# kishwarshafin/pepper

Measured on AMD Instinct MI355X. Metric: inference windows/sec (whole node), higher is better.
Workload: dtype f32 via f16 hi/lo split operands (3 MFMAs per product), f32 accumulate

## Files before the change

### include/pepper_amd_debug.h

```cpp
#ifndef PEPPER_AMD_DEBUG_H
#define PEPPER_AMD_DEBUG_H

#ifdef __cplusplus
extern "C" {
#endif

int pa_debug_dump_timing(unsigned long long* host_out);
int pa_debug_dump_gru_timing(unsigned long long* host_out);
void pa_debug_gemm_h2_experiment(int e);
int pa_debug_gemm_h2(const float* A, const float* W, const float* bias, float* C, int a_rows, int M, int N, int K, int act,
                     int frag_T, int frag_nb, int iters, float* ms_out);
int pa_debug_gemm_h2_split(const float* A, const float* W, const float* bias, float* C_new, float* C_parent, int a_rows, int M,
                           int N, int K, int act, int splits, int iters, float* ms_new, float* ms_parent);

#ifdef __cplusplus
}
#endif
#endif
```

### pepper_amd/csrc/api.hip

```cpp
#include "../../include/pepper_amd.h"

#include <hip/hip_runtime.h>

#include <algorithm>
#include <cmath>
#include <cstdio>
#include <cstdlib>
#include <cstring>
#include <map>
#include <string>
#include <vector>

#include "dec_frag16.h"
#include "kernels.h"

namespace {
thread_local std::string g_err;
}

namespace pa {
int set_error(int code, const std::string& msg) {
    g_err = msg;
    return code;
}
// ... 680 lines not shown
        HIP_TRY(hipMemsetAsync(m->us_failed->p, 0, sizeof(int), m->stream));
        HIP_TRY(hipMemcpyAsync(&m->us_host[1], ovf_counter, sizeof(int), hipMemcpyDeviceToHost, m->stream));
    }
    const size_t xp_bytes = std::max(s.need_xp ? (size_t)np * T * NX * sizeof(float) : (size_t)0,
                                     (size_t)8 * n * m->L1 * sizeof(float));
    if (int rc = m->xp->ensure(xp_bytes)) return rc;
    if (int rc = m->ya->ensure((size_t)np * T * 2 * H * sizeof(float))) return rc;
    if (m->rec.size() > 1)
        if (int rc = m->yb->ensure((size_t)np * T * 2 * H * sizeof(float))) return rc;
    if (int rc = m->l1->ensure((size_t)n * m->L1 * sizeof(float))) return rc;
    if (int rc = m->l2->ensure((size_t)n * m->L1 * sizeof(float))) return rc;
    const int tiles1 = (int)((n + 255) / 256) * ((m->L1 + 255) / 256);
    while (!bi && s.l1_splits < 32 && tiles1 * s.l1_splits * 2 <= 256 &&
           (size_t)(s.l1_splits * 2) * n * m->L1 * sizeof(float) <= m->xp->bytes)
        s.l1_splits *= 2;
    if (bi) s.l1_splits = kCanonicalL1Splits;

    const void* cur = images;
    int cur_kind = a_kind, cur_ld = F;
    bool cur_h2 = false;
    float* ybuf[2] = {m->ya->f(), m->yb->f()};
    int which = 0;
    const int M = (int)(n * T);
    for (size_t li = 0; li < m->rec.size(); ++li) {
        const RecLayer& r = m->rec[li];
        const LayerForm<Rec>& f = forms[li];
        float* y = ybuf[which];
        const float* bias_l = (f.y_h2 && r.prescaled) ? r.b_in_s->f() : r.b_in->f();
        const float* wih_l = (f.y_h2 && r.prescaled) ? r.w_ih_s->f() : r.w_ih->f();
        if (f.proj == XP_GEMM_H2) {
            const size_t a_bytes = (size_t)M * cur_ld * sizeof(float);
            if (!cur_h2)
                LAUNCH_TRY(m, "cvt_h2", 0.0,
                           pa::launch_f32_to_h2(static_cast<const float*>(cur), const_cast<void*>(cur), M, r.K,
                                                cur_ld, m->stream));
            LAUNCH_TRY(m, "gemm_h2_inproj", 2.0 * M * NX * r.K,
                       pa::launch_gemm_h2(cur, cur_ld, a_bytes, r.w_ih_h2->p, r.K, (size_t)NX * r.K * 4, bias_l,
                                          m->xp->f(), NX, (int)(np * T), NX, r.K, 0, 0, 0, T, (int)n, m->stream));
        } else if (f.proj == XP_GEMM_F32) {
            LAUNCH_TRY(m, li == 0 ? "gemm_inproj_in" : "gemm_inproj", 2.0 * M * NX * r.K,
                       pa::launch_gemm_nt(cur_kind, cur, cur_ld, wih_l, r.Kp, bias_l, m->xp->f(),
                                          NX, (int)(np * T), NX, r.K, 0, 0, 0, T, (int)n, m->stream));
        }
        switch (f.rec) {
        case FUSED_IN_H2:
            LAUNCH_TRY(m, "lstm_rec_h2_fused_in", 2.0 * n * T * (4.0 * H) * (H + r.K) * 2,
                       pa::launch_lstm_enc_h2(H, static_cast<const int8_t*>(cur), r.K, bias_l, r.w_cat_h2->p, y, 2 * H, (int)n, T,
                                              m->stream, s.small_rows));
            break;
        case FUSED_IN_F32:
            LAUNCH_TRY(m, "lstm_rec_fused_in", 2.0 * n * T * (4.0 * H) * (H + r.K) * 2,
                       pa::launch_lstm_rec_fused(H, static_cast<const int8_t*>(cur), r.K, r.b_in->f(),
                                                 r.w_cat->f(), y, 2 * H, (int)n, T, m->stream));
            break;
        case FUSED_DEC_H2:
            LAUNCH_TRY(m, "lstm_dec_h2_fused", 2.0 * n * T * (4.0 * H) * (H + r.K) * 2,
                       pa::launch_lstm_dec_h2(H, cur, cur_ld, bias_l, r.w_cat_dec_h2->p, y, 2 * H, (int)n, T, m->stream,
                                              bi && s.small_rows));
            break;
        case SPLIT_H2: {
            const int sabotage = m->split_sabotage > 0 ? 1 : 0;
            m->split_sabotage -= sabotage;
            LAUNCH_TRY(m, "lstm_rec_h2_split", 2.0 * n * T * (4.0 * H) * H * 2,
                       pa::launch_lstm_rec_h2_split(H, m->xp->f(), NX, r.w_hh_h2->p, y, 2 * H, (int)n, T, m->us_exch->p,
                                                    m->us_cnt->p, static_cast<int*>(m->us_failed->p), m->stream, sabotage));
            break;
        }
        case PLAIN_H2:
            LAUNCH_TRY(m, "lstm_rec_h2", 2.0 * n * T * (4.0 * H) * H * 2,
                       pa::launch_lstm_seed_h2(H, m->xp->f(), NX, r.w_hh_h2->p, y, 2 * H, (int)n, T, m->stream, s.small_rows));
            break;
        case PLAIN_F32:
            LAUNCH_TRY(m, "lstm_rec", 2.0 * n * T * (4.0 * H) * H * 2,
                       pa::launch_lstm_rec(H, m->xp->f(), NX, r.w_hh->f(), y, 2 * H, (int)n, T, m->stream));
            break;
        }
        cur = y;
        cur_kind = pa::A_F32;
        cur_ld = 2 * H;
        cur_h2 = f.y_h2;
        which ^= 1;
    }
    const int K1 = T * 2 * H;
    if (m->split_gemm && m->lin[0].w_h2 != nullptr && cur_kind == pa::A_F32) {
        if (!cur_h2)
            LAUNCH_TRY(m, "cvt_h2", 0.0,
                       pa::launch_f32_to_h2(static_cast<const float*>(cur), const_cast<void*>(cur), n, K1, K1, m->stream));
        LAUNCH_TRY(m, "gemm_h2_linear_1", 2.0 * n * m->L1 * K1,
                   pa::launch_gemm_h2(cur, K1, (size_t)n * K1 * 4, m->lin[0].w_h2->p, K1, (size_t)m->L1 * K1 * 4,
                                      m->lin[0].b->f(), m->l1->f(), m->L1, (int)n, m->L1, K1, 1, 0, 0, 0, 0, m->stream,
                                      s.l1_splits > 1 ? m->xp->f() : nullptr, s.l1_splits));
    } else {
        LAUNCH_TRY(m, "gemm_linear_1", 2.0 * n * m->L1 * K1,
                   pa::launch_gemm_nt(pa::A_F32, cur, K1, m->lin[0].w->f(), K1, m->lin[0].b->f(), m->l1->f(),
                                      m->L1, (int)n, m->L1, K1, 1, 0, 0, 0, 0, m->stream));
    }
    if (m->mlp_w != nullptr && C <= 8) {
        LAUNCH_TRY(m, "mlp_tail_h2", 2.0 * n * m->L1 * (4.0 * m->L1 + C),
                   pa::launch_mlp_tail_h2(m->l1->f(), m->L1, m->mlp_w->p, m->mlp_b->f(), 4, m->out.w->f(), m->out.b->f(), C,
                                          probs, logits, (int)n, m->stream, static_cast<const float* const*>(m->mlp_w32->p),
                                          ovf_counter, bi));
        if (s.unit_split) {
            HIP_TRY(hipMemcpyAsync(&m->us_host[0], m->us_failed->p, sizeof(int), hipMemcpyDeviceToHost, m->stream));
            HIP_TRY(hipStreamSynchronize(m->stream));
            if (m->us_host[0] != 0) {
                ++m->split_fallbacks;
                m->split_holdoff = US_HOLDOFF;
                HIP_TRY(hipMemcpyAsync(ovf_counter, &m->us_host[1], sizeof(int), hipMemcpyHostToDevice, m->stream));
                return variant_forward_chunk(m, a_kind, images, n, probs, logits, false);
            }
        }
        return PA_OK;
    }
    float* a = m->l1->f();
    float* b = m->l2->f();
    for (int i = 1; i < 5; ++i) {
        LAUNCH_TRY(m, "gemm_linear_2to5", 2.0 * n * m->L1 * m->L1,
                   pa::launch_gemm_nt(pa::A_F32, a, m->L1, m->lin[i].w->f(), m->L1, m->lin[i].b->f(), b,
                                      m->L1, (int)n, m->L1, m->L1, 1, 0, 0, 0, 0, m->stream));
        std::swap(a, b);
    }
    LAUNCH_TRY(m, "head_softmax", 2.0 * n * m->L1 * C,
               pa::launch_dense_small(0, a, m->L1, m->out.w->f(), m->out.b->f(), probs, logits, (int)n,
                                      m->L1, C, 1, 1, 0, m->stream));
    return PA_OK;
}

static int variant_forward(pa_variant_model* m, int a_kind, const void* images, size_t elem, int64_t n,
                           float* probs, float* logits) {
    if (!as_base(m)) return fail(PA_ERR_INVALID, "bad model handle");
    if (n < 0 || (n > 0 && (!images || !probs))) return fail(PA_ERR_INVALID, "null buffer");
    HIP_TRY(hipSetDevice(m->device));
    const int64_t per = (int64_t)m->cfg.window * m->cfg.image_features;
    const int C = m->cfg.num_classes_type;
    for (int64_t off = 0; off < n; off += m->cfg.max_chunk) {
        const int64_t c = std::min<int64_t>(m->cfg.max_chunk, n - off);
        const char* img = static_cast<const char*>(images) + (size_t)off * per * elem;
        if (int rc = variant_forward_chunk(m, a_kind, img, c, probs + off * C,
                                           logits ? logits + off * C : nullptr))
            return rc;
    }
    return PA_OK;
}

int pa_variant_split_fallbacks(pa_variant_model* m, int64_t* calls) {
    if (!as_base(m) || !calls) return fail(PA_ERR_INVALID, "bad argument");
    *calls = m->split_fallbacks;
    return PA_OK;
}

int pa_variant_set_batch_invariant(pa_variant_model* m, int32_t on) {
    return set_batch_invariant(m, on, "pa_variant_set_batch_invariant");
}

int pa_variant_get_batch_invariant(pa_variant_model* m, int32_t* on) { return get_batch_invariant(m, on); }

int pa_variant_overflow_rows(pa_variant_model* m, int64_t* rows) {
    if (!as_base(m) || !rows) return fail(PA_ERR_INVALID, "bad model handle");
    HIP_TRY(hipSetDevice(m->device));
    int v = 0;
    if (m->mlp_w32 != nullptr) {
        HIP_TRY(hipStreamSynchronize(m->stream));
        HIP_TRY(hipMemcpy(&v, m->ovf_counter(), sizeof(int), hipMemcpyDeviceToHost));
    }
    *rows = v;
    return PA_OK;
}

int pa_variant_forward_device(pa_variant_model* m, const int8_t* images, int64_t n, float* probs,
                              float* logits) {
    return variant_forward(m, pa::A_I8, images, 1, n, probs, logits);
}

int pa_variant_forward_device_f32(pa_variant_model* m, const float* images, int64_t n, float* probs,
                                  float* logits) {
    return variant_forward(m, pa::A_F32_SCALAR, images, 4, n, probs, logits);
}

int pa_variant_forward_host(pa_variant_model* m, const int8_t* images, int64_t n, float* probs,
                            float* logits) {
    if (!as_base(m)) return fail(PA_ERR_INVALID, "bad model handle");
    if (n < 0 || (n > 0 && (!images || !probs))) return fail(PA_ERR_INVALID, "null buffer");
    if (n == 0) return PA_OK;
    const size_t per = (size_t)m->cfg.window * m->cfg.image_features;
// ... 428 lines not shown
```

### pepper_amd/csrc/gemm_h2.hip

```cpp
#include "common.h"
#include "kernels.h"

#include <cstdlib>
#include <vector>

namespace {

typedef _Float16 h8 __attribute__((ext_vector_type(8)));

constexpr int HM = 256, HN = 256, HK = 32;
constexpr int HROW = 36;
constexpr int HSTAGE = (HM + HN) * HROW;

PA_DEV f32x16 mfma_h(h8 a, h8 b, f32x16 c) { return __builtin_amdgcn_mfma_f32_32x32x16_f16(a, b, c, 0, 0, 0); }

template <int ACT, int EXP = 0>
__global__ __launch_bounds__(256) void gemm_h2_kernel(const uint32_t* __restrict__ A, int lda, uint32_t a_bytes,
                                                      const uint32_t* __restrict__ W, int ldw, uint32_t w_bytes,
                                                      const float* __restrict__ bias, float* __restrict__ C, int ldc,
                                                      int M, int N, int K, int tiles_n, int nwg, int a_rpb,
                                                      int64_t a_bstride, int frag_T, int frag_nb) {
    __shared__ __attribute__((aligned(16))) uint32_t lds[2 * HSTAGE];

    const int tile = xcd_swizzle(blockIdx.x, nwg);
// ... 298 lines not shown
    int lane_ep = lane;
    asm volatile("" : "+v"(lane_ep));
    const int row_ep = m0 + wm * 128 + (lane_ep & 15), col_ep = n0 + wn * 128 + 4 * (lane_ep >> 4);
#pragma unroll
    for (int m = 0; m < 8; ++m) {
        const int row = row_ep + m * 16;
#pragma unroll
        for (int n = 0; n < 8; ++n) {
            const int col = col_ep + n * 16;
            if (row < M && col < N) *reinterpret_cast<f32x4*>(C + (size_t)row * N + col) = acc[m][n];
        }
    }
}

template <int ACT>
__global__ __launch_bounds__(256) void splitk_finish_kernel(const float* __restrict__ part, int S, const float* __restrict__ bias,
                                                            float* __restrict__ C, int ldc, int M, int N) {
    const size_t idx = (size_t)blockIdx.x * 256 + threadIdx.x;
    const int n4 = N >> 2;
    if (idx >= (size_t)M * n4) return;
    const int row = (int)(idx / n4), c = (int)(idx % n4) * 4;
    f32x4 v = *reinterpret_cast<const f32x4*>(part + (size_t)row * N + c);
    for (int s = 1; s < S; ++s) {
        const f32x4 w = *reinterpret_cast<const f32x4*>(part + ((size_t)s * M + row) * N + c);
        v += w;
    }
    if (bias != nullptr) v += *reinterpret_cast<const f32x4*>(bias + c);
    if (ACT == 1) { v.x = selu_f(v.x); v.y = selu_f(v.y); v.z = selu_f(v.z); v.w = selu_f(v.w); }
    *reinterpret_cast<f32x4*>(C + (size_t)row * ldc + c) = v;
}

__global__ __launch_bounds__(256) void f32_to_h2_kernel(const float* __restrict__ src, uint32_t* __restrict__ dst,
                                                        int64_t rows, int K, int64_t ld) {
    const int64_t idx = (int64_t)blockIdx.x * 256 + threadIdx.x;
    const int gpr = K >> 3;
    if (idx >= rows * gpr) return;
    const int64_t r = idx / gpr;
    const int g = (int)(idx - r * gpr);
    const float* s = src + r * ld + g * 8;
    h8 hi, lo;
#pragma unroll
    for (int e = 0; e < 8; ++e) {
        hi[e] = (_Float16)s[e];
        lo[e] = (_Float16)(s[e] - (float)hi[e]);
    }
    h8* d = reinterpret_cast<h8*>(dst + r * ld + g * 8);
    d[0] = hi;
    d[1] = lo;
}

}

namespace pa {

static bool g_h2_split_parent = false;
int g_h2_exp = 0;

void split_h2_host(const float* src, uint32_t* dst, int64_t rows, int K, int64_t ld_src, int64_t ld_dst) {
    for (int64_t r = 0; r < rows; ++r) {
        const float* s = src + r * ld_src;
        _Float16* d = reinterpret_cast<_Float16*>(dst + r * ld_dst);
        for (int g = 0; g < K / 8; ++g)
            for (int e = 0; e < 8; ++e) {
                const float v = s[g * 8 + e];
                const _Float16 hi = (_Float16)v;
                d[g * 16 + e] = hi;
                d[g * 16 + 8 + e] = (_Float16)(v - (float)hi);
            }
    }
}

hipError_t launch_f32_to_h2(const float* src, void* dst, int64_t rows, int K, int64_t ld, hipStream_t stream) {
    if ((K & 7) || (ld & 7)) return hipErrorInvalidValue;
    const int64_t n = rows * (K >> 3);
    if (n == 0) return hipSuccess;
    hipLaunchKernelGGL(f32_to_h2_kernel, dim3((unsigned)((n + 255) / 256)), dim3(256), 0, stream, src,
                       reinterpret_cast<uint32_t*>(dst), rows, K, ld);
    return hipGetLastError();
}

hipError_t launch_gemm_h2(const void* A, int lda, size_t a_bytes, const void* W, int ldw, size_t w_bytes,
                          const float* bias, float* C, int ldc, int M, int N, int K, int act, int a_rpb,
                          int64_t a_bstride, int frag_T, int frag_nb, hipStream_t stream, float* splitk_ws,
                          int splits) {
    if (frag_T > 0 && ((M & 31) || (N & 31) || act != 0)) return hipErrorInvalidValue;
    if ((K % HK) || (lda & 7) || (ldw & 7) || (a_bstride & 7) || ((uintptr_t)A & 15) || ((uintptr_t)W & 15))
        return hipErrorInvalidValue;
    if (a_bytes >= (1ull << 32) || w_bytes >= (1ull << 32)) return hipErrorInvalidValue;
    const int tiles_m = (M + HM - 1) / HM, tiles_n = (N + HN - 1) / HN;
    const int nwg = tiles_m * tiles_n;
    if (nwg == 0) return hipSuccess;
    const uint32_t* Au = reinterpret_cast<const uint32_t*>(A);
    const uint32_t* Wu = reinterpret_cast<const uint32_t*>(W);
    if (splits > 1 && splitk_ws != nullptr && frag_T == 0 && !(N & 3) && K / HK >= splits) {
        if (g_h2_split_parent)
            hipLaunchKernelGGL((gemm_h2_kernel<0>), dim3(nwg, splits), dim3(256), 0, stream, Au, lda, (uint32_t)a_bytes, Wu,
                               ldw, (uint32_t)w_bytes, (const float*)nullptr, splitk_ws, N, M, N, K, tiles_n, nwg, a_rpb,
                               a_bstride, 0, 0);
        else
            hipLaunchKernelGGL(gemm_h2_k32_kernel, dim3(nwg, splits), dim3(256), 0, stream, Au, lda, (uint32_t)a_bytes, Wu,
                               ldw, (uint32_t)w_bytes, splitk_ws, M, N, K, tiles_n, nwg, a_rpb, a_bstride);
        const size_t n4 = (size_t)M * (N >> 2);
        if (act == 1)
            hipLaunchKernelGGL((splitk_finish_kernel<1>), dim3((unsigned)((n4 + 255) / 256)), dim3(256), 0, stream,
                               splitk_ws, splits, bias, C, ldc, M, N);
        else
            hipLaunchKernelGGL((splitk_finish_kernel<0>), dim3((unsigned)((n4 + 255) / 256)), dim3(256), 0, stream,
                               splitk_ws, splits, bias, C, ldc, M, N);
        return hipGetLastError();
    }
    if (g_h2_exp > 0 && g_h2_exp < 8) {
#define PA_EXP(E_) case E_: hipLaunchKernelGGL((gemm_h2_kernel<0, E_>), dim3(nwg), dim3(256), 0, stream, Au, lda, (uint32_t)a_bytes, Wu, ldw, (uint32_t)w_bytes, bias, C, ldc, M, N, K, tiles_n, nwg, a_rpb, a_bstride, frag_T, frag_nb); break;
        switch (g_h2_exp) { PA_EXP(1) PA_EXP(2) PA_EXP(3) PA_EXP(4) PA_EXP(5) PA_EXP(6) PA_EXP(7) }
#undef PA_EXP
        return hipGetLastError();
    }
    if (act == 1)
        hipLaunchKernelGGL((gemm_h2_kernel<1>), dim3(nwg), dim3(256), 0, stream, Au, lda, (uint32_t)a_bytes, Wu, ldw,
                           (uint32_t)w_bytes, bias, C, ldc, M, N, K, tiles_n, nwg, a_rpb, a_bstride, frag_T, frag_nb);
    else
        hipLaunchKernelGGL((gemm_h2_kernel<0>), dim3(nwg), dim3(256), 0, stream, Au, lda, (uint32_t)a_bytes, Wu, ldw,
                           (uint32_t)w_bytes, bias, C, ldc, M, N, K, tiles_n, nwg, a_rpb, a_bstride, frag_T, frag_nb);
    return hipGetLastError();
}

}

extern "C" void pa_debug_gemm_h2_experiment(int e) { pa::g_h2_exp = e; }

extern "C" int pa_debug_gemm_h2(const float* A, const float* W, const float* bias, float* C, int a_rows, int M, int N,
                                int K, int act, int frag_T, int frag_nb, int iters, float* ms_out) {
    void *dA = nullptr, *dA2 = nullptr, *dW = nullptr, *dB = nullptr, *dC = nullptr;
    const size_t a_bytes = (size_t)a_rows * K * 4, w_bytes = (size_t)N * K * 4;
    const size_t c_elems = frag_T > 0 ? (size_t)M * N : (size_t)M * N;
    std::vector<uint32_t> wh((size_t)N * K);
    pa::split_h2_host(W, wh.data(), N, K, K, K);
    hipError_t e = hipSuccess;
    auto ok = [&](hipError_t r) { if (e == hipSuccess) e = r; return r == hipSuccess; };
    ok(hipMalloc(&dA, a_bytes)); ok(hipMalloc(&dA2, a_bytes)); ok(hipMalloc(&dW, w_bytes));
    ok(hipMalloc(&dB, (size_t)N * 4)); ok(hipMalloc(&dC, c_elems * 4));
    if (e == hipSuccess) {
        ok(hipMemcpy(dA, A, a_bytes, hipMemcpyHostToDevice));
        ok(hipMemcpy(dW, wh.data(), w_bytes, hipMemcpyHostToDevice));
        if (bias) ok(hipMemcpy(dB, bias, (size_t)N * 4, hipMemcpyHostToDevice));
        ok(hipMemset(dC, 0, c_elems * 4));
        ok(pa::launch_f32_to_h2((const float*)dA, dA2, a_rows, K, K, nullptr));
        hipEvent_t e0, e1;
        ok(hipEventCreate(&e0)); ok(hipEventCreate(&e1));
        ok(pa::launch_gemm_h2(dA2, K, a_bytes, dW, K, w_bytes, bias ? (const float*)dB : nullptr, (float*)dC, N, M, N, K,
                              act, 0, 0, frag_T, frag_nb, nullptr));
        ok(hipDeviceSynchronize());
        ok(hipEventRecord(e0, nullptr));
        for (int i = 0; i < iters; ++i)
            ok(pa::launch_gemm_h2(dA2, K, a_bytes, dW, K, w_bytes, bias ? (const float*)dB : nullptr, (float*)dC, N, M, N,
                                  K, act, 0, 0, frag_T, frag_nb, nullptr));
        ok(hipEventRecord(e1, nullptr));
        ok(hipEventSynchronize(e1));
        float ms = 0.0f;
        ok(hipEventElapsedTime(&ms, e0, e1));
        if (ms_out) *ms_out = iters > 0 ? ms / iters : 0.0f;
        ok(hipMemcpy(C, dC, c_elems * 4, hipMemcpyDeviceToHost));
        (void)hipEventDestroy(e0);
        (void)hipEventDestroy(e1);
    }
    for (void* p : {(void*)dA, (void*)dA2, (void*)dW, (void*)dB, (void*)dC}) (void)hipFree(p);
    if (e != hipSuccess) return pa::set_error((int)e, std::string("pa_debug_gemm_h2: ") + hipGetErrorString(e));
    return 0;
}

extern "C" int pa_debug_gemm_h2_split(const float* A, const float* W, const float* bias, float* C_new, float* C_parent,
                                      int a_rows, int M, int N, int K, int act, int splits, int iters, float* ms_new,
                                      float* ms_parent) {
    if (splits < 2 || (N & 3) || K % HK || K / HK < splits || a_rows < 1 || M < 1)
        return pa::set_error((int)hipErrorInvalidValue, "pa_debug_gemm_h2_split: needs splits >= 2, N % 4 == 0, K / 32 >= splits");
    void *dA = nullptr, *dA2 = nullptr, *dW = nullptr, *dB = nullptr, *dC = nullptr, *dWs = nullptr;
    const size_t a_bytes = (size_t)a_rows * K * 4, w_bytes = (size_t)N * K * 4, c_elems = (size_t)M * N;
    std::vector<uint32_t> wh((size_t)N * K);
    pa::split_h2_host(W, wh.data(), N, K, K, K);
    hipError_t e = hipSuccess;
    auto ok = [&](hipError_t r) { if (e == hipSuccess) e = r; return r == hipSuccess; };
    ok(hipMalloc(&dA, a_bytes)); ok(hipMalloc(&dA2, a_bytes)); ok(hipMalloc(&dW, w_bytes));
    ok(hipMalloc(&dB, (size_t)N * 4)); ok(hipMalloc(&dC, c_elems * 4)); ok(hipMalloc(&dWs, c_elems * 4 * splits));
    if (e == hipSuccess) {
        ok(hipMemcpy(dA, A, a_bytes, hipMemcpyHostToDevice));
// ... 33 lines not shown
```

### pepper_amd/csrc/kernels.h

```cpp
#pragma once
#include <hip/hip_runtime.h>
#include <stdint.h>

#include <string>

namespace pa {

int set_error(int code, const std::string& msg);

enum AKind { A_F32 = 0, A_I8 = 1, A_U8 = 2, A_F32_SCALAR = 3 };

hipError_t launch_gemm_nt(int a_type, const void* A, int lda, const float* W, int ldw,
                          const float* bias, float* C, int ldc, int M, int N, int K, int act,
                          int a_rpb, int64_t a_bstride, int frag_T, int frag_nb, hipStream_t stream);

hipError_t launch_gemm_h2(const void* A, int lda, size_t a_bytes, const void* W, int ldw, size_t w_bytes,
                          const float* bias, float* C, int ldc, int M, int N, int K, int act, int a_rpb,
                          int64_t a_bstride, int frag_T, int frag_nb, hipStream_t stream,
                          float* splitk_ws = nullptr, int splits = 1);
hipError_t launch_f32_to_h2(const float* src, void* dst, int64_t rows, int K, int64_t ld, hipStream_t stream);
void split_h2_host(const float* src, uint32_t* dst, int64_t rows, int K, int64_t ld_src, int64_t ld_dst);

hipError_t launch_lstm_rec(int H, const float* Xp, int ldx, const float* Wp, float* Y, int ldy,
                           int B, int T, hipStream_t stream);
hipError_t launch_lstm_rec_fused(int H, const int8_t* X, int F, const float* bias, const float* Wcat,
                                 float* Y, int ldy, int B, int T, hipStream_t stream);
hipError_t launch_gru_rec(int H, const float* Xp, int ldx, const float* Wp, const float* bhn,
                          const float* h0, int ldh0, float* hn, int ldhn, float* Y, int ldy,
                          int B, int T, hipStream_t stream);

hipError_t launch_gru_rec_fused(int H, const uint8_t* X, int F, int64_t x_bstride, const float* bias,
                                const float* Wcat, const float* bhn, const float* h0, int ldh0, float* hn, int ldhn,
                                float* Y, int ldy, int B, int T, hipStream_t stream);

void pack_rec_weights_h2(const float* const whh[2], const float* const wih[2], int G, int H, int F, int KX,
                         uint32_t* out, const float* const* bias = nullptr);
size_t rec_weights_h2_words(int G, int H, int KX);
int gru_fused_input_kx(int H, int F);
hipError_t launch_lstm_seed_h2(int H, const float* Xp, int ldx, const void* Wp, void* Y, int ldy, int B, int T,
                               hipStream_t stream, bool small = false);
hipError_t launch_lstm_enc_h2(int H, const int8_t* X, int F, const float* bias, const void* Wp, void* Y, int ldy, int B, int T,
                              hipStream_t stream, bool small = false);

size_t lstm_split_exchange_bytes(int B);
size_t lstm_split_counter_bytes(int B);
int lstm_split_grid(int B);
int lstm_split_resident_workgroups(int ntw);
hipError_t launch_lstm_rec_h2_split(int H, const float* Xp, int ldx, const void* Wp, void* Y, int ldy, int B, int T, void* exch,
                                    void* counters, int* failed, hipStream_t stream, int sabotage = 0);

hipError_t launch_lstm_dec_h2(int H, const void* Xh, int ldxh, const float* bias, const void* Wp, void* Y, int ldy, int B,
                              int T, hipStream_t stream, bool small = false);
hipError_t launch_gru_rec_h2(int H, const float* Xp, int ldx, const uint8_t* X, int F, int64_t x_bstride,
                             const float* bias, const void* Wp, const float* bhn, const float* h0, int ldh0, float* hn,
                             int ldhn, void* Y, int ldy, int B, int T, hipStream_t stream);

void pack_gru_small_weights_h2(const float* const whh[2], int H, uint32_t* out);
size_t gru_small_weights_h2_words(int H);
hipError_t launch_gru_small_h2(int H, const float* Xp, int ldx, const void* Wp, const float* bhn, const float* h0, int ldh0,
                               float* hn, int ldhn, void* Y, int ldy, int B, int T, hipStream_t stream);
hipError_t launch_gru_dec_h2(int H, const void* Xh, int ldxh, const float* bias, const void* Wp, const float* bhn,
                             const float* h0, int ldh0, float* hn, int ldhn, void* Y, int ldy, int B, int T,
                             hipStream_t stream);

void pack_dense_head_h2(const float* W, int C, int H, uint32_t* out);
size_t dense_head_h2_words(int H);
size_t dense_partials_floats(int B, int T);
hipError_t launch_gru_dec_h2_dense(int H, const void* Xh, int ldxh, const float* bias, const void* Wp, const float* bhn,
                                   const float* h0, int ldh0, float* hn, int ldhn, const void* Wd, float* P, int B, int T,
                                   hipStream_t stream);
hipError_t launch_polish_combine(const float* P, const float* bias, float* acc, int B, int T, int C, int S, int off,
                                 hipStream_t stream);

void pack_mlp_weights_h2(const float* const* W, int NL, uint32_t* out, float* scale);
size_t mlp_weights_h2_words(int NL);
hipError_t launch_mlp_tail_h2(const float* X, int ldx, const void* Wp, const float* bias, int NL, const float* Wout,
                              const float* bout, int C, float* probs, float* logits, int n, hipStream_t stream,
                              const float* const* W32, int* overflow_rows, bool per_row = false);

hipError_t launch_dense_small(int mode, const float* X, int ldx, const float* W, const float* bias,
                              float* out0, float* out1, int rows, int K, int C, int T, int S, int off,
                              hipStream_t stream);
hipError_t launch_polish_dense_acc_h2(const void* X, int ldx, const float* W, const float* bias, float* acc, int rows,
                                      int K, int C, int T, int S, int off, hipStream_t stream);
hipError_t launch_h2_to_f32(void* buf, int64_t rows, int K, int64_t ld, hipStream_t stream);
hipError_t launch_polish_finalize(const float* acc, uint8_t* labels, uint8_t* phred, int64_t B, int S,
                                  int C, int overlap, hipStream_t stream);

void launch_bgzf_inflate(hipStream_t stream, const uint8_t* comp, const int64_t* comp_off, const int32_t* comp_len,
                         const int64_t* out_off, const int32_t* out_len, uint8_t* out, int32_t* status, int n_blocks,
                         int64_t comp_bytes, unsigned long long* debug_counts = nullptr);
const char* inflate_status_text(int32_t s);
void launch_record_walk(hipStream_t stream, const uint8_t* data, int64_t data_bytes, const int64_t* entries, int n_entries, int cap,
                        void* slots, int32_t* counts, int32_t* base, int32_t* flags, void* out, int64_t out_cap, int32_t* tail,
                        int split = 0);
}
```

### pepper_amd/csrc/mlp_h2.hip

```cpp
#include "common.h"
#include "kernels.h"

namespace {

typedef _Float16 h8 __attribute__((ext_vector_type(8)));

constexpr int MT = 64, D = 512, KS = D / 16, NTILES = D / 32;
constexpr int ROWB = D * 4 + 16, ROWD = ROWB / 4;

PA_DEV f32x16 mfma_h(h8 a, h8 b, f32x16 c) { return __builtin_amdgcn_mfma_f32_32x32x16_f16(a, b, c, 0, 0, 0); }

template <int NL, bool PERROW = false>
__global__ __launch_bounds__(512, 1) void mlp_tail_h2_kernel(const float* __restrict__ X, int ldx,
                                                             const uint32_t* __restrict__ Wp,
                                                             const float* __restrict__ bias,
                                                             const float* __restrict__ Wout,
                                                             const float* __restrict__ bout, int C,
                                                             float* __restrict__ probs, float* __restrict__ logits,
                                                             int n, const float* const* __restrict__ W32,
                                                             int* __restrict__ overflow_rows) {
    extern __shared__ __attribute__((aligned(16))) uint32_t lds[];
    static_assert((ROWB / 16) % 2 == 1, "row stride must be an odd number of 16-byte slots");
    const int tid = threadIdx.x, lane = tid & 63;
    const int w = __builtin_amdgcn_readfirstlane(tid >> 6);
    const int li = lane & 31, hf = lane >> 5;
    const int b0 = blockIdx.x * MT;

    bool bad = false;
    uint32_t* rowbad = lds + MT * ROWD;
    {
        const int row = tid >> 3, gsel = tid & 7;
        int grow = b0 + row;
        grow = grow < n ? grow : n - 1;
        const float* src = X + (size_t)grow * ldx;
#pragma unroll
        for (int j = 0; j < 8; ++j) {
            const int g = gsel + 8 * j;
            const f32x4 a = *reinterpret_cast<const f32x4*>(src + g * 8);
            const f32x4 b = *reinterpret_cast<const f32x4*>(src + g * 8 + 4);
            const float v[8] = {a.x, a.y, a.z, a.w, b.x, b.y, b.z, b.w};
            h8 hi, lo;
#pragma unroll
            for (int e = 0; e < 8; ++e) {
                bad |= !(fabsf(v[e]) < 65504.0f);
                hi[e] = (_Float16)v[e];
                lo[e] = (_Float16)(v[e] - (float)hi[e]);
            }
            *reinterpret_cast<h8*>(lds + row * ROWD + g * 8) = hi;
            *reinterpret_cast<h8*>(lds + row * ROWD + g * 8 + 4) = lo;
        }
        if (PERROW) {
            int b8 = bad ? 1 : 0;
            b8 |= __shfl_xor(b8, 1, 64);
            b8 |= __shfl_xor(b8, 2, 64);
            b8 |= __shfl_xor(b8, 4, 64);
            if (gsel == 0) rowbad[row] = (uint32_t)b8;
        }
    }
    __syncthreads();

    const uint32_t* arow = lds + li * ROWD + hf * 8;
    const bool odd = li & 1;
    struct Frag { h8 b[2][2], a[2][2]; };

#pragma unroll 1
    for (int layer = 0; layer < NL; ++layer) {
        const __amdgpu_buffer_rsrc_t wrs = __builtin_amdgcn_make_buffer_rsrc(
            const_cast<uint32_t*>(Wp + ((size_t)layer * NTILES + 2 * w) * KS * 512), 0, 0x7fffffff, 0x00020000);
        const unsigned woff = lane * 16u;
        auto load_step = [&](int s, Frag& fr) {
#pragma unroll
            for (int nn = 0; nn < 2; ++nn)
#pragma unroll
                for (int hl = 0; hl < 2; ++hl)
                    fr.b[nn][hl] = __builtin_bit_cast(h8, __builtin_amdgcn_raw_buffer_load_b128(
                                                              wrs, woff, (unsigned)((nn * KS + s) * 2 + hl) * 1024u, 0));
#pragma unroll
            for (int m = 0; m < 2; ++m) {
                fr.a[m][0] = *reinterpret_cast<const h8*>(arow + m * 32 * ROWD + s * 16);
                fr.a[m][1] = *reinterpret_cast<const h8*>(arow + m * 32 * ROWD + s * 16 + 4);
            }
        };
        f32x16 acc[2][2];
#pragma unroll
        for (int nn = 0; nn < 2; ++nn) {
            const float bv = bias[layer * D + 64 * w + 32 * nn + li];
#pragma unroll
            for (int m = 0; m < 2; ++m)
#pragma unroll
                for (int r = 0; r < 16; ++r) acc[m][nn][r] = bv;
        }
        Frag ring[2];
        load_step(0, ring[0]);
#pragma unroll
        for (int s = 0; s < KS; ++s) {
            const int p = s & 1;
            if (s + 1 < KS) load_step(s + 1, ring[p ^ 1]);
#pragma unroll
            for (int term = 0; term < 3; ++term)
#pragma unroll
                for (int nn = 0; nn < 2; ++nn)
#pragma unroll
                    for (int m = 0; m < 2; ++m)
                        acc[m][nn] = mfma_h(ring[p].a[m][term == 0 ? 1 : 0], ring[p].b[nn][term == 1 ? 1 : 0], acc[m][nn]);
            if (s + 1 < KS) {
#pragma unroll
                for (int q = 0; q < 4; ++q) {
                    __builtin_amdgcn_sched_group_barrier(0x008, 1, 0);
                    __builtin_amdgcn_sched_group_barrier(0x020, 1, 0);
                }
#pragma unroll
                for (int q = 0; q < 4; ++q) {
                    __builtin_amdgcn_sched_group_barrier(0x008, 1, 0);
                    __builtin_amdgcn_sched_group_barrier(0x100, 1, 0);
                }
                __builtin_amdgcn_sched_group_barrier(0x008, 4, 0);
            }
            __builtin_amdgcn_sched_barrier(0);
        }
        lds_barrier();
        const float unscale = bias[NL * D + layer];
#pragma unroll
        for (int nn = 0; nn < 2; ++nn) {
            const int col = 64 * w + 32 * nn + li;
            uint32_t* dst = lds + 4 * hf * ROWD + (col >> 3) * 8 + (odd ? 4 : 0) + ((col & 7) >> 1);
#pragma unroll
            for (int m = 0; m < 2; ++m)
#pragma unroll
                for (int r = 0; r < 16; ++r) {
                    const float v = selu_f(acc[m][nn][r] * unscale);
                    bad |= !(fabsf(v) < 65504.0f);
                    if (PERROW && !(fabsf(v) < 65504.0f)) rowbad[4 * hf + 32 * m + (r & 3) + 8 * (r >> 2)] = 1u;
                    dst[(32 * m + (r & 3) + 8 * (r >> 2)) * ROWD] = h2_word_of(v, h2_select(odd));
                }
        }
        lds_barrier();
    }

    float* frow = reinterpret_cast<float*>(lds);
    auto head = [&](bool from_f32, bool select) {
        float wo[8][8];
#pragma unroll
        for (int c = 0; c < 8; ++c)
#pragma unroll
            for (int e = 0; e < 8; ++e) wo[c][e] = c < C ? Wout[(size_t)c * D + lane * 8 + e] : 0.0f;
        for (int rr = 0; rr < 8; ++rr) {
            const int row = 8 * w + rr;
            if (PERROW && select && (rowbad[row] != 0) != from_f32) continue;
            const h8 hi = *reinterpret_cast<const h8*>(lds + row * ROWD + lane * 8);
            const h8 lo = *reinterpret_cast<const h8*>(lds + row * ROWD + lane * 8 + 4);
            float x[8];
#pragma unroll
            for (int e = 0; e < 8; ++e) x[e] = from_f32 ? frow[row * ROWD + lane * 8 + e] : (float)hi[e] + (float)lo[e];
            float logit[8], mx = -INFINITY;
#pragma unroll
            for (int c = 0; c < 8; ++c) {
                float p = 0.0f;
#pragma unroll
                for (int e = 0; e < 8; ++e) p += x[e] * wo[c][e];
#pragma unroll
                for (int o = 32; o > 0; o >>= 1) p += __shfl_xor(p, o, 64);
                logit[c] = c < C ? p + bout[c < C ? c : 0] : -INFINITY;
                mx = fmaxf(mx, logit[c]);
            }
            float e[8], den = 0.0f;
#pragma unroll
            for (int c = 0; c < 8; ++c) {
                e[c] = c < C ? expf(logit[c] - mx) : 0.0f;
                den += e[c];
            }
            float my_logit = 0.0f, my_e = 0.0f;
#pragma unroll
            for (int c = 0; c < 8; ++c)
                if (lane == c) { my_logit = logit[c]; my_e = e[c]; }
            const int grow = b0 + row;
            if (grow < n && lane < C) {
                probs[(size_t)grow * C + lane] = my_e / den;
                if (logits != nullptr) logits[(size_t)grow * C + lane] = my_logit;
            }
        }
    };

    const bool rerun = __syncthreads_or(bad ? 1 : 0) != 0;
    if (PERROW) {
        head(false, rerun);
        if (rerun) __syncthreads();
    }
    if (rerun) {
        if (tid == 0 && overflow_rows != nullptr) {
            int cnt = n - b0 < MT ? n - b0 : MT;
            if (PERROW) {
                cnt = 0;
                for (int r = 0; r < MT && b0 + r < n; ++r) cnt += rowbad[r] != 0 ? 1 : 0;
            }
            atomicAdd(overflow_rows, cnt);
        }
        for (int i = tid; i < MT * D; i += 512) {
            const int row = i / D, col = i - row * D;
            const int grow = b0 + row < n ? b0 + row : n - 1;
            frow[row * ROWD + col] = X[(size_t)grow * ldx + col];
        }
        __syncthreads();
#pragma unroll 1
        for (int layer = 0; layer < NL; ++layer) {
            const float* wr = W32[layer] + (size_t)tid * D;
            float y[MT];
            const float bv = bias[NL * D + NL + layer * D + tid];
#pragma unroll
            for (int r = 0; r < MT; ++r) y[r] = bv;
#pragma unroll 1
            for (int k = 0; k < D; k += 4) {
                const f32x4 wv = *reinterpret_cast<const f32x4*>(wr + k);
#pragma unroll
                for (int r = 0; r < MT; ++r) {
                    const f32x4 xv = *reinterpret_cast<const f32x4*>(frow + r * ROWD + k);
                    y[r] = fmaf(xv.x, wv.x, y[r]);
                    y[r] = fmaf(xv.y, wv.y, y[r]);
                    y[r] = fmaf(xv.z, wv.z, y[r]);
                    y[r] = fmaf(xv.w, wv.w, y[r]);
                }
            }
            __syncthreads();
#pragma unroll
            for (int r = 0; r < MT; ++r) frow[r * ROWD + tid] = selu_f(y[r]);
            __syncthreads();
        }
    }

    if (PERROW) {
        if (rerun) head(true, true);
    } else {
        head(rerun, false);
    }
}

}

namespace pa {

void pack_mlp_weights_h2(const float* const* W, int NL, uint32_t* out, float* scale) {
    _Float16* o = reinterpret_cast<_Float16*>(out);
    for (int l = 0; l < NL; ++l) {
        float mx = 0.0f;
        for (size_t i = 0; i < (size_t)D * D; ++i) mx = fmaxf(mx, fabsf(W[l][i]));
        int e = 0;
        if (mx > 0.0f) {
            (void)frexpf(mx, &e);
            e = 14 - e;
            e = e > 60 ? 60 : (e < -60 ? -60 : e);
        }
        const float sc = ldexpf(1.0f, e);
        scale[l] = sc;
        for (int nt = 0; nt < NTILES; ++nt)
            for (int s = 0; s < KS; ++s)
                for (int ln = 0; ln < 64; ++ln)
                    for (int e8 = 0; e8 < 8; ++e8) {
                        const float v = sc * W[l][(size_t)(nt * 32 + (ln & 31)) * D + 16 * s + 8 * (ln >> 5) + e8];
                        const _Float16 hi = (_Float16)v;
                        const size_t base = ((((size_t)l * NTILES + nt) * KS + s) * 2) * 512 + (size_t)ln * 8 + e8;
                        o[base] = hi;
                        o[base + 512] = (_Float16)(v - (float)hi);
                    }
    }
}

size_t mlp_weights_h2_words(int NL) { return (size_t)NL * NTILES * KS * 2 * 256; }

hipError_t launch_mlp_tail_h2(const float* X, int ldx, const void* Wp, const float* bias, int NL, const float* Wout,
                              const float* bout, int C, float* probs, float* logits, int n, hipStream_t stream,
                              const float* const* W32, int* overflow_rows, bool per_row) {
    if (n <= 0) return hipSuccess;
    if (NL != 4 || C > 8 || C <= 0 || (ldx & 3) || W32 == nullptr) return hipErrorInvalidValue;
    if (per_row) {
        const size_t lds = (size_t)MT * ROWB + (size_t)MT * sizeof(uint32_t);
        hipLaunchKernelGGL((mlp_tail_h2_kernel<4, true>), dim3((n + MT - 1) / MT), dim3(512), lds, stream, X, ldx,
                           static_cast<const uint32_t*>(Wp), bias, Wout, bout, C, probs, logits, n, W32, overflow_rows);
        return hipGetLastError();
    }
    const size_t lds = (size_t)MT * ROWB;
    hipLaunchKernelGGL((mlp_tail_h2_kernel<4>), dim3((n + MT - 1) / MT), dim3(512), lds, stream, X, ldx,
                       static_cast<const uint32_t*>(Wp), bias, Wout, bout, C, probs, logits, n, W32, overflow_rows);
    return hipGetLastError();
}

}
```

Measured before the change: 2.880 million.

## Fuse split-K finish of linear_1 into MLP tail kernel; batch head rows

When linear_1 uses two split-K slices, the separate split-K finish kernel is skipped. The MLP tail now reads both partial slices plus the bias and applies SELU while loading its input rows. This removes one kernel launch and a full write and read of the L1 activation, at the cost of reading two partial buffers in the tail. The output head is also restructured to process four rows at a time with a compile-time class count (3 or 8), which batches the shuffle reductions. Optional debug timestamps are added and compiled out by default.

```diff
diff --git a/include/pepper_amd_debug.h b/include/pepper_amd_debug.h
--- a/include/pepper_amd_debug.h
+++ b/include/pepper_amd_debug.h
@@ -7,6 +7,7 @@
 
 int pa_debug_dump_timing(unsigned long long* host_out);
 int pa_debug_dump_gru_timing(unsigned long long* host_out);
+int pa_debug_dump_tail_timing(unsigned long long* host_out);
 void pa_debug_gemm_h2_experiment(int e);
 int pa_debug_gemm_h2(const float* A, const float* W, const float* bias, float* C, int a_rows, int M, int N, int K, int act,
                      int frag_T, int frag_nb, int iters, float* ms_out);
diff --git a/pepper_amd/csrc/api.hip b/pepper_amd/csrc/api.hip
--- a/pepper_amd/csrc/api.hip
+++ b/pepper_amd/csrc/api.hip
@@ -786,6 +786,8 @@
         which ^= 1;
     }
     const int K1 = T * 2 * H;
+    static_assert(kCanonicalL1Splits == 2, "mlp_tail_h2_kernel's PARTS form adds two slices");
+    bool l1_parts = PA_TAIL_FROM_PARTS && s.l1_splits == kCanonicalL1Splits && m->mlp_w != nullptr && C <= 8 && m->L1 == 512;
     if (m->split_gemm && m->lin[0].w_h2 != nullptr && cur_kind == pa::A_F32) {
         if (!cur_h2)
             LAUNCH_TRY(m, "cvt_h2", 0.0,
@@ -793,17 +795,19 @@
         LAUNCH_TRY(m, "gemm_h2_linear_1", 2.0 * n * m->L1 * K1,
                    pa::launch_gemm_h2(cur, K1, (size_t)n * K1 * 4, m->lin[0].w_h2->p, K1, (size_t)m->L1 * K1 * 4,
                                       m->lin[0].b->f(), m->l1->f(), m->L1, (int)n, m->L1, K1, 1, 0, 0, 0, 0, m->stream,
-                                      s.l1_splits > 1 ? m->xp->f() : nullptr, s.l1_splits));
+                                      s.l1_splits > 1 ? m->xp->f() : nullptr, s.l1_splits, &l1_parts));
     } else {
+        l1_parts = false;
         LAUNCH_TRY(m, "gemm_linear_1", 2.0 * n * m->L1 * K1,
                    pa::launch_gemm_nt(pa::A_F32, cur, K1, m->lin[0].w->f(), K1, m->lin[0].b->f(), m->l1->f(),
                                       m->L1, (int)n, m->L1, K1, 1, 0, 0, 0, 0, m->stream));
     }
     if (m->mlp_w != nullptr && C <= 8) {
         LAUNCH_TRY(m, "mlp_tail_h2", 2.0 * n * m->L1 * (4.0 * m->L1 + C),
-                   pa::launch_mlp_tail_h2(m->l1->f(), m->L1, m->mlp_w->p, m->mlp_b->f(), 4, m->out.w->f(), m->out.b->f(), C,
-                                          probs, logits, (int)n, m->stream, static_cast<const float* const*>(m->mlp_w32->p),
-                                          ovf_counter, bi));
+                   pa::launch_mlp_tail_h2(l1_parts ? m->xp->f() : m->l1->f(), m->L1, m->mlp_w->p, m->mlp_b->f(), 4, m->out.w->f(),
+                                          m->out.b->f(), C, probs, logits, (int)n, m->stream,
+                                          static_cast<const float* const*>(m->mlp_w32->p), ovf_counter, bi,
+                                          l1_parts ? m->lin[0].b->f() : nullptr, l1_parts ? (size_t)n * m->L1 : 0));
         if (s.unit_split) {
             HIP_TRY(hipMemcpyAsync(&m->us_host[0], m->us_failed->p, sizeof(int), hipMemcpyDeviceToHost, m->stream));
             HIP_TRY(hipStreamSynchronize(m->stream));
diff --git a/pepper_amd/csrc/gemm_h2.hip b/pepper_amd/csrc/gemm_h2.hip
--- a/pepper_amd/csrc/gemm_h2.hip
+++ b/pepper_amd/csrc/gemm_h2.hip
@@ -404,7 +404,9 @@
 hipError_t launch_gemm_h2(const void* A, int lda, size_t a_bytes, const void* W, int ldw, size_t w_bytes,
                           const float* bias, float* C, int ldc, int M, int N, int K, int act, int a_rpb,
                           int64_t a_bstride, int frag_T, int frag_nb, hipStream_t stream, float* splitk_ws,
-                          int splits) {
+                          int splits, bool* leave_finish) {
+    const bool no_finish = leave_finish != nullptr && *leave_finish;
+    if (leave_finish != nullptr) *leave_finish = false;
     if (frag_T > 0 && ((M & 31) || (N & 31) || act != 0)) return hipErrorInvalidValue;
     if ((K % HK) || (lda & 7) || (ldw & 7) || (a_bstride & 7) || ((uintptr_t)A & 15) || ((uintptr_t)W & 15))
         return hipErrorInvalidValue;
@@ -422,6 +424,10 @@
         else
             hipLaunchKernelGGL(gemm_h2_k32_kernel, dim3(nwg, splits), dim3(256), 0, stream, Au, lda, (uint32_t)a_bytes, Wu,
                                ldw, (uint32_t)w_bytes, splitk_ws, M, N, K, tiles_n, nwg, a_rpb, a_bstride);
+        if (no_finish) {
+            *leave_finish = true;
+            return hipGetLastError();
+        }
         const size_t n4 = (size_t)M * (N >> 2);
         if (act == 1)
             hipLaunchKernelGGL((splitk_finish_kernel<1>), dim3((unsigned)((n4 + 255) / 256)), dim3(256), 0, stream,
diff --git a/pepper_amd/csrc/kernels.h b/pepper_amd/csrc/kernels.h
--- a/pepper_amd/csrc/kernels.h
+++ b/pepper_amd/csrc/kernels.h
@@ -17,7 +17,8 @@
 hipError_t launch_gemm_h2(const void* A, int lda, size_t a_bytes, const void* W, int ldw, size_t w_bytes,
                           const float* bias, float* C, int ldc, int M, int N, int K, int act, int a_rpb,
                           int64_t a_bstride, int frag_T, int frag_nb, hipStream_t stream,
-                          float* splitk_ws = nullptr, int splits = 1);
+                          float* splitk_ws = nullptr, int splits = 1,
+                          bool* leave_finish = nullptr);
 hipError_t launch_f32_to_h2(const float* src, void* dst, int64_t rows, int K, int64_t ld, hipStream_t stream);
 void split_h2_host(const float* src, uint32_t* dst, int64_t rows, int K, int64_t ld_src, int64_t ld_dst);
 
@@ -76,7 +77,11 @@
 size_t mlp_weights_h2_words(int NL);
 hipError_t launch_mlp_tail_h2(const float* X, int ldx, const void* Wp, const float* bias, int NL, const float* Wout,
                               const float* bout, int C, float* probs, float* logits, int n, hipStream_t stream,
-                              const float* const* W32, int* overflow_rows, bool per_row = false);
+                              const float* const* W32, int* overflow_rows, bool per_row = false,
+                              const float* l1_bias = nullptr, size_t part_stride = 0);
+#ifndef PA_TAIL_FROM_PARTS
+#define PA_TAIL_FROM_PARTS 1
+#endif
 
 hipError_t launch_dense_small(int mode, const float* X, int ldx, const float* W, const float* bias,
                               float* out0, float* out1, int rows, int K, int C, int T, int S, int off,
diff --git a/pepper_amd/csrc/mlp_h2.hip b/pepper_amd/csrc/mlp_h2.hip
--- a/pepper_amd/csrc/mlp_h2.hip
+++ b/pepper_amd/csrc/mlp_h2.hip
@@ -1,3 +1,5 @@
+#include <type_traits>
+
 #include "common.h"
 #include "kernels.h"
 
@@ -10,21 +12,53 @@
 
 PA_DEV f32x16 mfma_h(h8 a, h8 b, f32x16 c) { return __builtin_amdgcn_mfma_f32_32x32x16_f16(a, b, c, 0, 0, 0); }
 
-template <int NL, bool PERROW = false>
+#ifndef PA_DEBUG_TIMING
+#define PA_DEBUG_TIMING 0
+#endif
+constexpr int TAIL_STAMPS = 32;
+#if PA_DEBUG_TIMING
+#define PA_TAIL_STAMP(slot_)                                                                            \
+    do {                                                                                                \
+        __builtin_amdgcn_sched_barrier(0);                                                              \
+        unsigned long long t_;                                                                          \
+        asm volatile("s_memtime %0\n\ts_waitcnt lgkmcnt(0)" : "=s"(t_) : : "memory");                   \
+        __builtin_amdgcn_sched_barrier(0);                                                              \
+        if (stamp) dbg[w * TAIL_STAMPS + (slot_)] = t_;                                                 \
+    } while (0)
+#else
+#define PA_TAIL_STAMP(slot_) do { } while (0)
+#endif
+
+PA_DEV float l1_finish(float p0, float p1, float b) {
+    float v = p0;
+    v += p1;
+    v += b;
+    v = selu_f(v);
+    asm volatile("" : "+v"(v));
+    return v;
+}
+
+template <int NL, bool PERROW = false, bool PARTS = false>
 __global__ __launch_bounds__(512, 1) void mlp_tail_h2_kernel(const float* __restrict__ X, int ldx,
+                                                             const float* __restrict__ b1, size_t pstride,
                                                              const uint32_t* __restrict__ Wp,
                                                              const float* __restrict__ bias,
                                                              const float* __restrict__ Wout,
                                                              const float* __restrict__ bout, int C,
                                                              float* __restrict__ probs, float* __restrict__ logits,
                                                              int n, const float* const* __restrict__ W32,
-                                                             int* __restrict__ overflow_rows) {
+                                                             int* __restrict__ overflow_rows,
+                                                             unsigned long long* __restrict__ dbg) {
     extern __shared__ __attribute__((aligned(16))) uint32_t lds[];
     static_assert((ROWB / 16) % 2 == 1, "row stride must be an odd number of 16-byte slots");
     const int tid = threadIdx.x, lane = tid & 63;
     const int w = __builtin_amdgcn_readfirstlane(tid >> 6);
     const int li = lane & 31, hf = lane >> 5;
     const int b0 = blockIdx.x * MT;
+#if PA_DEBUG_TIMING
+    const bool stamp = dbg != nullptr && blockIdx.x == (gridDim.x > 8 ? 8u : 0u) && lane == 0;
+#endif
+    PA_TAIL_STAMP(0);
 
     bool bad = false;
     uint32_t* rowbad = lds + MT * ROWD;
@@ -33,12 +67,7 @@
         int grow = b0 + row;
         grow = grow < n ? grow : n - 1;
         const float* src = X + (size_t)grow * ldx;
-#pragma unroll
-        for (int j = 0; j < 8; ++j) {
-            const int g = gsel + 8 * j;
-            const f32x4 a = *reinterpret_cast<const f32x4*>(src + g * 8);
-            const f32x4 b = *reinterpret_cast<const f32x4*>(src + g * 8 + 4);
-            const float v[8] = {a.x, a.y, a.z, a.w, b.x, b.y, b.z, b.w};
+        auto split8 = [&](int g, const float (&v)[8]) {
             h8 hi, lo;
 #pragma unroll
             for (int e = 0; e < 8; ++e) {
@@ -48,6 +77,39 @@
             }
             *reinterpret_cast<h8*>(lds + row * ROWD + g * 8) = hi;
             *reinterpret_cast<h8*>(lds + row * ROWD + g * 8 + 4) = lo;
+        };
+        if (PARTS) {
+            const float* src1 = src + pstride;
+#pragma unroll
+            for (int jh = 0; jh < 2; ++jh) {
+                f32x4 p[4][3][2];
+#pragma unroll
+                for (int j = 0; j < 4; ++j) {
+                    const int c = (gsel + 8 * (4 * jh + j)) * 8;
+#pragma unroll
+                    for (int q = 0; q < 2; ++q) {
+                        p[j][0][q] = *reinterpret_cast<const f32x4*>(src + c + 4 * q);
+                        p[j][1][q] = *reinterpret_cast<const f32x4*>(src1 + c + 4 * q);
+                        p[j][2][q] = *reinterpret_cast<const f32x4*>(b1 + c + 4 * q);
+                    }
+                }
+#pragma unroll
+                for (int j = 0; j < 4; ++j) {
+                    float v[8];
+#pragma unroll
+                    for (int e = 0; e < 8; ++e) v[e] = l1_finish(p[j][0][e >> 2][e & 3], p[j][1][e >> 2][e & 3], p[j][2][e >> 2][e & 3]);
+                    split8(gsel + 8 * (4 * jh + j), v);
+                }
+            }
+        } else {
+#pragma unroll
+            for (int j = 0; j < 8; ++j) {
+                const int g = gsel + 8 * j;
+                const f32x4 a = *reinterpret_cast<const f32x4*>(src + g * 8);
+                const f32x4 b = *reinterpret_cast<const f32x4*>(src + g * 8 + 4);
+                const float v[8] = {a.x, a.y, a.z, a.w, b.x, b.y, b.z, b.w};
+                split8(g, v);
+            }
         }
         if (PERROW) {
             int b8 = bad ? 1 : 0;
@@ -58,6 +120,7 @@
         }
     }
     __syncthreads();
+    PA_TAIL_STAMP(1);
 
     const uint32_t* arow = lds + li * ROWD + hf * 8;
     const bool odd = li & 1;
@@ -118,7 +181,9 @@
             }
             __builtin_amdgcn_sched_barrier(0);
         }
+        PA_TAIL_STAMP(2 + 4 * layer);
         lds_barrier();
+        PA_TAIL_STAMP(3 + 4 * layer);
         const float unscale = bias[NL * D + layer];
 #pragma unroll
         for (int nn = 0; nn < 2; ++nn) {
@@ -134,51 +199,86 @@
                     dst[(32 * m + (r & 3) + 8 * (r >> 2)) * ROWD] = h2_word_of(v, h2_select(odd));
                 }
         }
+        PA_TAIL_STAMP(4 + 4 * layer);
         lds_barrier();
+        PA_TAIL_STAMP(5 + 4 * layer);
     }
 
     float* frow = reinterpret_cast<float*>(lds);
-    auto head = [&](bool from_f32, bool select) {
-        float wo[8][8];
-#pragma unroll
-        for (int c = 0; c < 8; ++c)
-#pragma unroll
-            for (int e = 0; e < 8; ++e) wo[c][e] = c < C ? Wout[(size_t)c * D + lane * 8 + e] : 0.0f;
-        for (int rr = 0; rr < 8; ++rr) {
-            const int row = 8 * w + rr;
-            if (PERROW && select && (rowbad[row] != 0) != from_f32) continue;
-            const h8 hi = *reinterpret_cast<const h8*>(lds + row * ROWD + lane * 8);
-            const h8 lo = *reinterpret_cast<const h8*>(lds + row * ROWD + lane * 8 + 4);
+    auto head_rows = [&](auto cc, auto rc, const float (&wo)[decltype(cc)::value][8], int row0, bool from_f32) __attribute__((always_inline)) {
+        constexpr int CC = decltype(cc)::value, R = decltype(rc)::value;
+        float p[R][CC];
+#pragma unroll
+        for (int j = 0; j < R; ++j) {
+            const int row = row0 + j;
             float x[8];
-#pragma unroll
-            for (int e = 0; e < 8; ++e) x[e] = from_f32 ? frow[row * ROWD + lane * 8 + e] : (float)hi[e] + (float)lo[e];
-            float logit[8], mx = -INFINITY;
-#pragma unroll
-            for (int c = 0; c < 8; ++c) {
-                float p = 0.0f;
-#pragma unroll
-                for (int e = 0; e < 8; ++e) p += x[e] * wo[c][e];
-#pragma unroll
-                for (int o = 32; o > 0; o >>= 1) p += __shfl_xor(p, o, 64);
-                logit[c] = c < C ? p + bout[c < C ? c : 0] : -INFINITY;
+            if (from_f32) {
+#pragma unroll
+                for (int e = 0; e < 8; ++e) x[e] = frow[row * ROWD + lane * 8 + e];
+            } else {
+                const h8 hi = *reinterpret_cast<const h8*>(lds + row * ROWD + lane * 8);
+                const h8 lo = *reinterpret_cast<const h8*>(lds + row * ROWD + lane * 8 + 4);
+#pragma unroll
+                for (int e = 0; e < 8; ++e) x[e] = (float)hi[e] + (float)lo[e];
+            }
+#pragma unroll
+            for (int c = 0; c < CC; ++c) {
+                p[j][c] = 0.0f;
+#pragma unroll
+                for (int e = 0; e < 8; ++e) p[j][c] += x[e] * wo[c][e];
+            }
+        }
+#pragma unroll
+        for (int o = 32; o > 0; o >>= 1)
+#pragma unroll
+            for (int j = 0; j < R; ++j)
+#pragma unroll
+                for (int c = 0; c < CC; ++c) p[j][c] += __shfl_xor(p[j][c], o, 64);
+#pragma unroll
+        for (int j = 0; j < R; ++j) {
+            float logit[CC], mx = -INFINITY;
+#pragma unroll
+            for (int c = 0; c < CC; ++c) {
+                logit[c] = c < C ? p[j][c] + bout[c < C ? c : 0] : -INFINITY;
                 mx = fmaxf(mx, logit[c]);
             }
-            float e[8], den = 0.0f;
-#pragma unroll
-            for (int c = 0; c < 8; ++c) {
+            float e[CC], den = 0.0f;
+#pragma unroll
+            for (int c = 0; c < CC; ++c) {
                 e[c] = c < C ? expf(logit[c] - mx) : 0.0f;
                 den += e[c];
             }
             float my_logit = 0.0f, my_e = 0.0f;
 #pragma unroll
-            for (int c = 0; c < 8; ++c)
+            for (int c = 0; c < CC; ++c)
                 if (lane == c) { my_logit = logit[c]; my_e = e[c]; }
-            const int grow = b0 + row;
+            const int grow = b0 + row0 + j;
             if (grow < n && lane < C) {
                 probs[(size_t)grow * C + lane] = my_e / den;
                 if (logits != nullptr) logits[(size_t)grow * C + lane] = my_logit;
             }
         }
+    };
+    auto head_cc = [&](auto cc, bool from_f32, bool select) __attribute__((always_inline)) {
+        constexpr int CC = decltype(cc)::value;
+        float wo[CC][8];
+#pragma unroll
+        for (int c = 0; c < CC; ++c)
+#pragma unroll
+            for (int e = 0; e < 8; ++e) wo[c][e] = c < C ? Wout[(size_t)c * D + lane * 8 + e] : 0.0f;
+        if (PERROW && select) {
+            for (int rr = 0; rr < 8; ++rr) {
+                const int row = 8 * w + rr;
+                if ((rowbad[row] != 0) != from_f32) continue;
+                head_rows(cc, std::integral_constant<int, 1>{}, wo, row, from_f32);
+            }
+        } else {
+            for (int rr = 0; rr < 8; rr += 4) head_rows(cc, std::integral_constant<int, 4>{}, wo, 8 * w + rr, from_f32);
+        }
+    };
+    auto head = [&](bool from_f32, bool select) __attribute__((always_inline)) {
+        if (C <= 3) head_cc(std::integral_constant<int, 3>{}, from_f32, select);
+        else head_cc(std::integral_constant<int, 8>{}, from_f32, select);
     };
 
     const bool rerun = __syncthreads_or(bad ? 1 : 0) != 0;
@@ -198,7 +298,8 @@
         for (int i = tid; i < MT * D; i += 512) {
             const int row = i / D, col = i - row * D;
             const int grow = b0 + row < n ? b0 + row : n - 1;
-            frow[row * ROWD + col] = X[(size_t)grow * ldx + col];
+            const size_t at = (size_t)grow * ldx + col;
+            frow[row * ROWD + col] = PARTS ? l1_finish(X[at], X[at + pstride], b1[col]) : X[at];
         }
         __syncthreads();
 #pragma unroll 1
@@ -232,6 +333,7 @@
     } else {
         head(rerun, false);
     }
+    PA_TAIL_STAMP(18);
 }
 
 }
@@ -266,21 +368,50 @@
 
 size_t mlp_weights_h2_words(int NL) { return (size_t)NL * NTILES * KS * 2 * 256; }
 
+#if PA_DEBUG_TIMING
+static unsigned long long* g_dbg_tail = nullptr;
+static unsigned long long* tail_debug_buffer() {
+    if (!g_dbg_tail) {
+        if (hipMalloc(&g_dbg_tail, 8 * TAIL_STAMPS * sizeof(unsigned long long)) != hipSuccess) return nullptr;
+        (void)hipMemset(g_dbg_tail, 0, 8 * TAIL_STAMPS * sizeof(unsigned long long));
+    }
+    return g_dbg_tail;
+}
+#else
+static unsigned long long* tail_debug_buffer() { return nullptr; }
+#endif
+
 hipError_t launch_mlp_tail_h2(const float* X, int ldx, const void* Wp, const float* bias, int NL, const float* Wout,
                               const float* bout, int C, float* probs, float* logits, int n, hipStream_t stream,
-                              const float* const* W32, int* overflow_rows, bool per_row) {
+                              const float* const* W32, int* overflow_rows, bool per_row, const float* l1_bias,
+                              size_t part_stride) {
     if (n <= 0) return hipSuccess;
     if (NL != 4 || C > 8 || C <= 0 || (ldx & 3) || W32 == nullptr) return hipErrorInvalidValue;
-    if (per_row) {
-        const size_t lds = (size_t)MT * ROWB + (size_t)MT * sizeof(uint32_t);
-        hipLaunchKernelGGL((mlp_tail_h2_kernel<4, true>), dim3((n + MT - 1) / MT), dim3(512), lds, stream, X, ldx,
-                           static_cast<const uint32_t*>(Wp), bias, Wout, bout, C, probs, logits, n, W32, overflow_rows);
-        return hipGetLastError();
-    }
-    const size_t lds = (size_t)MT * ROWB;
-    hipLaunchKernelGGL((mlp_tail_h2_kernel<4>), dim3((n + MT - 1) / MT), dim3(512), lds, stream, X, ldx,
-                       static_cast<const uint32_t*>(Wp), bias, Wout, bout, C, probs, logits, n, W32, overflow_rows);
+    const bool parts = l1_bias != nullptr;
+    if (parts && (ldx != D || part_stride < (size_t)n * D || (part_stride & 3))) return hipErrorInvalidValue;
+    const size_t lds = (size_t)MT * ROWB + (per_row ? (size_t)MT * sizeof(uint32_t) : 0);
+    const dim3 grid((n + MT - 1) / MT), block(512);
+    const uint32_t* Wu = static_cast<const uint32_t*>(Wp);
+    unsigned long long* dbg = tail_debug_buffer();
+#define PA_TAIL_LAUNCH(PERROW_, PARTS_)                                                                                          \
+    hipLaunchKernelGGL((mlp_tail_h2_kernel<4, PERROW_, PARTS_>), grid, block, lds, stream, X, ldx, l1_bias, part_stride, Wu, bias, \
+                       Wout, bout, C, probs, logits, n, W32, overflow_rows, dbg)
+    if (per_row && parts) PA_TAIL_LAUNCH(true, true);
+    else if (per_row) PA_TAIL_LAUNCH(true, false);
+    else if (parts) PA_TAIL_LAUNCH(false, true);
+    else PA_TAIL_LAUNCH(false, false);
+#undef PA_TAIL_LAUNCH
     return hipGetLastError();
 }
 
 }
+
+extern "C" int pa_debug_dump_tail_timing(unsigned long long* host_out) {
+#if PA_DEBUG_TIMING
+    if (!pa::g_dbg_tail) return 1;
+    return hipMemcpy(host_out, pa::g_dbg_tail, 8 * TAIL_STAMPS * sizeof(unsigned long long), hipMemcpyDeviceToHost) == hipSuccess ? 0 : 2;
+#else
+    (void)host_out;
+    return 1;
+#endif
+}
```

New measurement: 2.890 million, median of 2. About the same (+0.3%).
